# nelaturuharsha/TurboPrune

Measured on NVIDIA H100. Metric: images_per_sec_resnet50_erk80_train_step, higher is better.
Workload: dtype bf16

## Files before the change

turboprune_b200/csrc/tp_igemm.cu:

```cuda
#include "tp_common.cuh"
#include "tp_ptx.cuh"
#include <cuda.h>
#include <mutex>

namespace tp {
using namespace ptx;

constexpr int kBlockM = 128;
constexpr int kBlockK = 64;
constexpr int kConsumers = 256;
constexpr int kThreads = kConsumers + 32;
constexpr int kProducerWarp = kConsumers / 32;
constexpr int kMaxTaps = 64;

__host__ __device__ constexpr int fwd_stages(int block_n) { return block_n == 128 ? 4 : 6; }
__host__ __device__ constexpr int fwd_tail(int block_n) { return kBlockM * block_n * 4 + 8 * 32 * 128 + 1024 + 512; }

struct TapEntry { uint16_t off_w, off_h; int32_t kofs; };

constexpr int kMaxCls = 4;

struct ClsEntry {
  int M;
  int P_it, Q_it;
  int ntaps, tap0;
  int base_w, base_h;
  int oah, oaw;
  int tile0, m_groups;
};

struct FwdParams {
  int M, N;
  int ncls;
  ClsEntry cls[kMaxCls];
  int cchunks;
  int a_mode;
  int step_w, step_h;
  long long out_img_pix;
  int out_row_pix;
// ... 70 lines not shown
  const int ntile = p.m_tiles * p.n_tiles;
  w.split = item / ntile;
  const int tile = item - w.split * ntile, n_t = tile / p.m_tiles;
  w.set_tile(tile - n_t * p.m_tiles, n_t, p.m_tiles, nb, p.chunks);
  w.kb0 = w.split * p.kb_per_split; w.kb1 = min(p.kblocks, w.kb0 + p.kb_per_split);
  return w;
}

__device__ __forceinline__ void decompose_pixel(int m, int P, int Q, int& n, int& p, int& q) {
  q = m % Q; int t = m / Q; p = t % P; n = t / P;
}

struct AMaps { CUtensorMap m[kMaxCls]; };

__device__ __forceinline__ void decode_tile(const FwdParams& p, int tile, int n_tiles, int& c, int& m_g, int& n_t) {
  c = 0;
#pragma unroll
  for (int j = 1; j < kMaxCls; ++j) if (j < p.ncls && tile >= p.cls[j].tile0) c = j;
  const int local = tile - p.cls[c].tile0;
  m_g = local / n_tiles; n_t = local - m_g * n_tiles;
}

template <int BLOCK_N>
__device__ __forceinline__ void fwd_mma_block(float (&acc)[BLOCK_N / 2], uint32_t a_addr, uint32_t b_addr, uint32_t accumulate) {
  const uint64_t adesc = make_smem_desc(a_addr, 16, 1024);
  const uint64_t bdesc = make_smem_desc(b_addr, 16, 1024);
#pragma unroll
  for (int k = 0; k < kBlockK / 16; ++k) {
    if constexpr (BLOCK_N == 128) wgmma_m64n128<0, 0>(acc, adesc + (uint64_t)(2 * k), bdesc + (uint64_t)(2 * k), accumulate | (uint32_t)k);
    else wgmma_m64n64<0, 0>(acc, adesc + (uint64_t)(2 * k), bdesc + (uint64_t)(2 * k), accumulate | (uint32_t)k);
  }
}

template <int BLOCK_N, bool MULTI, bool BNB>
__global__ void __launch_bounds__(kThreads, 1)
k_igemm_fwd(const __grid_constant__ AMaps tmA, const __grid_constant__ CUtensorMap tmB,
            const __grid_constant__ FwdParams p) {
  static_assert(BLOCK_N == 64 || BLOCK_N == 128, "wgmma N of the fwd kernel");
  static_assert(!BNB || !MULTI, "BatchNorm-backward epilogue: single class");
  constexpr int kABytes = kBlockM * kBlockK * 2;
  constexpr int kBBytes = BLOCK_N * kBlockK * 2;
  constexpr int kStageBytes = kABytes + kBBytes;
  constexpr int kStages = fwd_stages(BLOCK_N);
  extern __shared__ __align__(1024) uint8_t smem_raw[];
  uint8_t* smem = (uint8_t*)(((uintptr_t)smem_raw + 1023) & ~(uintptr_t)1023);
  pdl_trigger();
  constexpr int kStgBytes = 32 * 128;
  float* const acc_tile = (float*)(smem + kStages * kStageBytes);
  uint8_t* stg_base = (uint8_t*)(acc_tile + kBlockM * BLOCK_N);
  uint64_t* full_bar = (uint64_t*)(stg_base + 8 * kStgBytes);
  uint64_t* empty_bar = full_bar + kStages;

  const int warp = threadIdx.x >> 5, lane = threadIdx.x & 31;
  const int n_tiles = (p.N + BLOCK_N - 1) / BLOCK_N;
  const int total_tiles = p.cls[p.ncls - 1].tile0 + p.cls[p.ncls - 1].m_groups * n_tiles;
  const int my_items = total_tiles > (int)blockIdx.x ? (total_tiles - (int)blockIdx.x + (int)gridDim.x - 1) / (int)gridDim.x : 0;
  auto get_tile = [&](int w, int& ci, int& m_g, int& n_t) {
    ci = 0;
    const int tile = (int)blockIdx.x + w * (int)gridDim.x;
    if (MULTI) decode_tile(p, tile, n_tiles, ci, m_g, n_t);
    else { m_g = tile / n_tiles; n_t = tile - m_g * n_tiles; }
  };

  if (threadIdx.x == 0) {
    for (int j = 0; j < p.ncls; ++j) prefetch_tmap(&tmA.m[j]);
    prefetch_tmap(&tmB);
    for (int i = 0; i < kStages; ++i) { mbar_init(&full_bar[i], 1); mbar_init(&empty_bar[i], kConsumers / 128); }
    fence_mbar_init();
  }
  __syncthreads();
  pdl_wait();

  if (warp == kProducerWarp) {
    if (lane == 0) {
      int stage = 0; uint32_t phase = 0;
      const uint32_t* const km = live_kmask(p.kmask, p.kmask_words, p.N);
      for (int w = 0; w < my_items; ++w) {
        int ci, m_g, n_t; get_tile(w, ci, m_g, n_t);
        const ClsEntry& ce = p.cls[MULTI ? ci : 0];
        const CUtensorMap* const mapA = &tmA.m[MULTI ? ci : 0];
        const int m0 = m_g * kBlockM;
        int cn = 0, cp = 0, cq = 0;
        if (p.a_mode == 1) decompose_pixel(m0, ce.P_it, ce.Q_it, cn, cp, cq);
        const int cw = ce.base_w + cq * p.step_w, ch = ce.base_h + cp * p.step_h;
        auto load_block = [&](const TapEntry& te, int cc) {
          mbar_wait(&empty_bar[stage], phase ^ 1);
          uint8_t* sA = smem + stage * kStageBytes;
          uint8_t* sB = sA + kABytes;
          mbar_arrive_expect_tx(&full_bar[stage], kStageBytes);
          if (p.a_mode == 1)
            tma_load_im2col_4d(sA, mapA, &full_bar[stage], cc * kBlockK, cw, ch, cn, te.off_w, te.off_h);
          else
            tma_load_2d(sA, mapA, &full_bar[stage], te.kofs + cc * kBlockK, m0);
          tma_load_2d(sB, &tmB, &full_bar[stage], te.kofs + cc * kBlockK, n_t * BLOCK_N);
          if (++stage == kStages) { stage = 0; phase ^= 1; }
        };
        const int tap_base = MULTI ? ce.tap0 : 0;
        if (!km) {
          for (int tap = 0; tap < ce.ntaps; ++tap) {
            const TapEntry te = p.taps[tap_base + tap];
            for (int cc = 0; cc < p.cchunks; ++cc) load_block(te, cc);
          }
        } else {
          KSkip ks; bool any = false;
          ks.begin(km, p.kmask_words, n_t * BLOCK_N, BLOCK_N, p.N);
          for (int tap = 0; tap < ce.ntaps; ++tap) {
            const TapEntry te = p.taps[tap_base + tap];
            for (int cc = 0; cc < p.cchunks; ++cc) {
              const bool last = tap == ce.ntaps - 1 && cc == p.cchunks - 1;
              if (!ks.take((te.kofs >> 6) + cc, last, any)) continue;
              any = true;
              load_block(te, cc);
            }
          }
        }
      }
    }
  } else {
    const int wg = warp >> 2;
    const int quarter = warp & 3;
    const int half = warp >> 2;
    const int erow = quarter * 32 + lane;
    int stage = 0; uint32_t phase = 0;
    const uint32_t* const km = live_kmask(p.kmask, p.kmask_words, p.N);
    auto acc_row_ld = [&](int c, uint32_t* v) {
      const uint32_t rb = smem_u32(acc_tile) + (uint32_t)(erow * BLOCK_N * 4);
#pragma unroll
      for (int i = 0; i < 8; ++i) {
        const uint4 t = lds128(rb + ((uint32_t)(((c >> 2) + i) ^ (erow & 7)) << 4));
        v[4 * i] = t.x; v[4 * i + 1] = t.y; v[4 * i + 2] = t.z; v[4 * i + 3] = t.w;
      }
    };
    for (int w = 0; w < my_items; ++w) {
      int ci, m_g, n_t; get_tile(w, ci, m_g, n_t);
      const ClsEntry& ce = p.cls[MULTI ? ci : 0];
      const bool has_acc = MULTI ? ce.ntaps > 0 : true;
      const int m_t = m_g;
      const int row = m_t * kBlockM + quarter * 32 + lane;
      const bool row_ok = row < ce.M;
      long long opix = 0;
      if (row_ok && !p.staged_store) {
        opix = row;
        if (MULTI || !p.linear) {
          int n, pp, qq; decompose_pixel(row, ce.P_it, ce.Q_it, n, pp, qq);
          opix = (long long)n * p.out_img_pix + (long long)(pp * p.osh + ce.oah) * p.out_row_pix + (qq * p.osw + ce.oaw);
        }
      }
      __nv_bfloat16* orow = p.out + opix * p.ldc;
      const int r_in = lane >> 3, c16 = lane & 7;
      const long long wrow0 = (long long)m_t * kBlockM + quarter * 32;
      const int rows_left = (int)(ce.M - wrow0 < 32 ? (ce.M - wrow0 < 0 ? 0 : ce.M - wrow0) : 32);
      const long long ldc = p.ldc;
      const int N = p.N;
      long long ooff[MULTI ? 8 : 1];
      const long long rbase = (wrow0 + r_in) * ldc + c16 * 8;
      if (MULTI && p.staged_store) {
        int n, pp, qq; decompose_pixel((int)(wrow0 + r_in), ce.P_it, ce.Q_it, n, pp, qq);
#pragma unroll
        for (int i = 0; i < 8; ++i) {
          const long long px = (long long)n * p.out_img_pix + (long long)(pp * p.osh + ce.oah) * p.out_row_pix + (qq * p.osw + ce.oaw);
          ooff[i] = px * ldc + c16 * 8;
          qq += 4;
          while (qq >= ce.Q_it) { qq -= ce.Q_it; if (++pp == ce.P_it) { pp = 0; ++n; } }
        }
      }
      auto row_off = [&](int i) -> long long { return MULTI ? ooff[MULTI ? i : 0] : rbase + (long long)(i * 4) * ldc; };
      if (MULTI && !has_acc) {
        if (p.staged_store) {
#pragma unroll 1
          for (int c = half * 64; c < BLOCK_N; c += 128) {
            const int n0 = n_t * BLOCK_N + c;
            if (n0 >= N) break;
            if (n0 + c16 * 8 + 8 > N) continue;
            uint4 z[8];
#pragma unroll
            for (int i = 0; i < 8; ++i) {
              z[i] = make_uint4(0u, 0u, 0u, 0u);
              if (p.addend && i * 4 + r_in < rows_left) z[i] = *reinterpret_cast<const uint4*>(p.addend + row_off(i) + n0);
            }
#pragma unroll
            for (int i = 0; i < 8; ++i)
              if (i * 4 + r_in < rows_left) *reinterpret_cast<uint4*>(p.out + row_off(i) + n0) = z[i];
          }
        } else if (row_ok && half == 0) {
          for (int j = n_t * BLOCK_N; j < min(p.N, (n_t + 1) * BLOCK_N); ++j)
            orow[j] = p.addend ? p.addend[opix * p.ldc + j] : __float2bfloat16_rn(0.f);
        }
        continue;
      }
      {
        float acc[BLOCK_N / 2];
#pragma unroll
        for (int i = 0; i < BLOCK_N / 2; ++i) acc[i] = 0.f;
        int prev = -1;
        auto mma_block = [&](uint32_t accumulate) {
          mbar_wait(&full_bar[stage], phase);
          const uint32_t s_addr = smem_u32(smem + stage * kStageBytes);
          wgmma_fence();
          fwd_mma_block<BLOCK_N>(acc, s_addr + (uint32_t)(wg * (kABytes / 2)), s_addr + kABytes, accumulate);
          wgmma_commit();
          wgmma_wait<1>();
          if (prev >= 0 && (threadIdx.x & 127) == 0) mbar_arrive(&empty_bar[prev]);
          prev = stage;
          if (++stage == kStages) { stage = 0; phase ^= 1; }
        };
        KSkip ks; uint32_t any = 0;
        if (km) ks.begin(km, p.kmask_words, n_t * BLOCK_N, BLOCK_N, p.N);
        for (int tap = 0; tap < ce.ntaps; ++tap) {
          const int kb0 = p.taps[(MULTI ? ce.tap0 : 0) + tap].kofs >> 6;
          for (int cc = 0; cc < p.cchunks; ++cc) {
            const bool last = tap == ce.ntaps - 1 && cc == p.cchunks - 1;
            if (km && !ks.take(kb0 + cc, last, any)) continue;
            mma_block(any);
            any = 1;
          }
        }
        wgmma_wait<0>();
        acc_fence(acc);
        if (prev >= 0 && (threadIdx.x & 127) == 0) mbar_arrive(&empty_bar[prev]);
        bar_sync(1, kConsumers);
        const int r0 = wg * 64 + (warp & 3) * 16 + (lane >> 2);
#pragma unroll
        for (int j = 0; j < BLOCK_N / 8; ++j)
#pragma unroll
          for (int h = 0; h < 2; ++h) {
            const int r = r0 + 8 * h, col = 8 * j + 2 * (lane & 3);
            *reinterpret_cast<float2*>(acc_tile + r * BLOCK_N + (((col >> 2) ^ (r & 7)) << 2) + (col & 3)) =
                make_float2(acc[4 * j + 2 * h], acc[4 * j + 2 * h + 1]);
          }
        bar_sync(1, kConsumers);
      }
      if (p.staged_store) {
        const uint32_t buf = smem_u32(stg_base + warp * kStgBytes);
        __nv_bfloat16* const gout = p.out;
        const __nv_bfloat16* const gadd = p.addend;
        const float* bias = p.bias;
        float* stats = p.stats ? p.stats + (long long)(m_t * 4 + quarter) * 2 * N + c16 * 8 : nullptr;
        const uint32_t wr_base = buf + lane * 128;
        const uint32_t wr_sw = (uint32_t)(lane & 7);
        const uint32_t rd_even = buf + r_in * 128 + ((uint32_t)(c16 ^ r_in) << 4);
        const uint32_t rd_odd = buf + (r_in + 4) * 128 + ((uint32_t)(c16 ^ (r_in + 4)) << 4);
        uint4 a_pref[8];
#pragma unroll 1
        for (int c = half * 64; c < BLOCK_N; c += 128) {
          const int n0 = n_t * BLOCK_N + c;
          if (n0 >= N) break;
          const bool col_ok = n0 + c16 * 8 + 8 <= N;
          uint32_t v[64];
          acc_row_ld(c, v);
          acc_row_ld(c + 32, v + 32);
          if (gadd) {
            if (c == half * 64) {
#pragma unroll
              for (int i = 0; i < 8; ++i) {
                a_pref[i] = make_uint4(0u, 0u, 0u, 0u);
                if (i * 4 + r_in < rows_left && col_ok) a_pref[i] = *reinterpret_cast<const uint4*>(gadd + row_off(i) + n0);
              }
            }
#pragma unroll
            for (int i = 0; i < 8; ++i) sts128(((i & 1) ? rd_odd : rd_even) + (uint32_t)((i >> 1) * 1024), a_pref[i]);
            if (c + 128 < BLOCK_N && n0 + 128 < N) {
              const bool col_ok2 = n0 + 128 + c16 * 8 + 8 <= N;
#pragma unroll
              for (int i = 0; i < 8; ++i) {
                a_pref[i] = make_uint4(0u, 0u, 0u, 0u);
                if (i * 4 + r_in < rows_left && col_ok2) a_pref[i] = *reinterpret_cast<const uint4*>(gadd + row_off(i) + n0 + 128);
              }
            }
            __syncwarp();
          }
#pragma unroll
          for (int j = 0; j < 64; j += 8) {
            float f[8];
#pragma unroll
            for (int q = 0; q < 8; ++q) f[q] = __uint_as_float(v[j + q]);
            if (bias) {
#pragma unroll
              for (int q = 0; q < 8; ++q) if (n0 + j + q < N) f[q] += bias[n0 + j + q];
            }
            const uint32_t waddr = wr_base + (((uint32_t)(j >> 3) ^ wr_sw) << 4);
            if (gadd) {
              const uint4 a = lds128(waddr);
              const __nv_bfloat162* ah = reinterpret_cast<const __nv_bfloat162*>(&a);
#pragma unroll
              for (int q = 0; q < 4; ++q) { const float2 t2 = __bfloat1622float2(ah[q]); f[2 * q] += t2.x; f[2 * q + 1] += t2.y; }
            }
            __nv_bfloat162 h0 = __floats2bfloat162_rn(f[0], f[1]);
            __nv_bfloat162 h1 = __floats2bfloat162_rn(f[2], f[3]);
            __nv_bfloat162 h2 = __floats2bfloat162_rn(f[4], f[5]);
            __nv_bfloat162 h3 = __floats2bfloat162_rn(f[6], f[7]);
            uint4 pk;
            pk.x = *(uint32_t*)&h0; pk.y = *(uint32_t*)&h1; pk.z = *(uint32_t*)&h2; pk.w = *(uint32_t*)&h3;
            sts128(waddr, pk);
          }
          __syncwarp();
          uint4 o[8];
#pragma unroll
          for (int i = 0; i < 8; ++i) o[i] = lds128(((i & 1) ? rd_odd : rd_even) + (uint32_t)((i >> 1) * 1024));
          float s1[8], s2[8];
#pragma unroll
          for (int q = 0; q < 8; ++q) { s1[q] = 0.f; s2[q] = 0.f; }
          if (BNB) {
            uint4 yv[8];
#pragma unroll
            for (int i = 0; i < 8; ++i) {
              yv[i] = make_uint4(0u, 0u, 0u, 0u);
              if (i * 4 + r_in < rows_left && col_ok) yv[i] = *reinterpret_cast<const uint4*>(p.bn_y + row_off(i) + n0);
            }
            float sc[8], sf[8], is_[8], nm[8];
            if (col_ok) {
              const int cb = n0 + c16 * 8;
#pragma unroll
              for (int q = 0; q < 8; q += 4) {
                const float4 one4 = make_float4(1.f, 1.f, 1.f, 1.f), zero4 = make_float4(0.f, 0.f, 0.f, 0.f);
                const float4 a4 = p.bn_weight ? *reinterpret_cast<const float4*>(p.bn_weight + cb + q) : one4;
                const float4 b4 = p.bn_bias ? *reinterpret_cast<const float4*>(p.bn_bias + cb + q) : zero4;
                const float4 m4 = *reinterpret_cast<const float4*>(p.bn_mean + cb + q), i4 = *reinterpret_cast<const float4*>(p.bn_invstd + cb + q);
                is_[q] = i4.x; is_[q + 1] = i4.y; is_[q + 2] = i4.z; is_[q + 3] = i4.w;
                nm[q] = m4.x; nm[q + 1] = m4.y; nm[q + 2] = m4.z; nm[q + 3] = m4.w;
                sc[q] = a4.x * i4.x; sc[q + 1] = a4.y * i4.y; sc[q + 2] = a4.z * i4.z; sc[q + 3] = a4.w * i4.w;
                sf[q] = fmaf(-m4.x, sc[q], b4.x); sf[q + 1] = fmaf(-m4.y, sc[q + 1], b4.y);
                sf[q + 2] = fmaf(-m4.z, sc[q + 2], b4.z); sf[q + 3] = fmaf(-m4.w, sc[q + 3], b4.w);
              }
            } else {
#pragma unroll
              for (int q = 0; q < 8; ++q) { sc[q] = 0.f; sf[q] = 0.f; is_[q] = 0.f; nm[q] = 0.f; }
            }
#pragma unroll
            for (int i = 0; i < 8; ++i) {
              if (i * 4 + r_in < rows_left) {
                __nv_bfloat162* gh = reinterpret_cast<__nv_bfloat162*>(&o[i]);
                const __nv_bfloat162* yh = reinterpret_cast<const __nv_bfloat162*>(&yv[i]);
#pragma unroll
                for (int q = 0; q < 4; ++q) {
                  float2 d2 = __bfloat1622float2(gh[q]);
                  const float2 y2 = __bfloat1622float2(yh[q]);
                  if (!(fmaf(y2.x, sc[2 * q], sf[2 * q]) > 0.f)) d2.x = 0.f;
                  if (!(fmaf(y2.y, sc[2 * q + 1], sf[2 * q + 1]) > 0.f)) d2.y = 0.f;
                  gh[q] = __floats2bfloat162_rn(d2.x, d2.y);
                  s1[2 * q] += d2.x;     s2[2 * q] = fmaf(d2.x, (y2.x - nm[2 * q]) * is_[2 * q], s2[2 * q]);
                  s1[2 * q + 1] += d2.y; s2[2 * q + 1] = fmaf(d2.y, (y2.y - nm[2 * q + 1]) * is_[2 * q + 1], s2[2 * q + 1]);
                }
              }
            }
          }
#pragma unroll
          for (int i = 0; i < 8; ++i)
            if (i * 4 + r_in < rows_left && col_ok) *reinterpret_cast<uint4*>(gout + row_off(i) + n0) = o[i];
          if (!BNB && stats) {
#pragma unroll
            for (int i = 0; i < 8; ++i) {
              if (i * 4 + r_in < rows_left) {
                const __nv_bfloat162* h2 = reinterpret_cast<const __nv_bfloat162*>(&o[i]);
#pragma unroll
                for (int q = 0; q < 4; ++q) {
                  const float2 t2 = __bfloat1622float2(h2[q]);
                  s1[2 * q] += t2.x; s2[2 * q] = fmaf(t2.x, t2.x, s2[2 * q]);
                  s1[2 * q + 1] += t2.y; s2[2 * q + 1] = fmaf(t2.y, t2.y, s2[2 * q + 1]);
                }
              }
            }
          }
          if (BNB || stats) {
#pragma unroll
            for (int q = 0; q < 8; ++q) {
              s1[q] += __shfl_xor_sync(0xffffffffu, s1[q], 8);  s2[q] += __shfl_xor_sync(0xffffffffu, s2[q], 8);
              s1[q] += __shfl_xor_sync(0xffffffffu, s1[q], 16); s2[q] += __shfl_xor_sync(0xffffffffu, s2[q], 16);
            }
            if (r_in == 0 && col_ok) {
              float4* d1 = reinterpret_cast<float4*>(stats + n0);
              float4* d2 = reinterpret_cast<float4*>(stats + N + n0);
              d1[0] = make_float4(s1[0], s1[1], s1[2], s1[3]); d1[1] = make_float4(s1[4], s1[5], s1[6], s1[7]);
              d2[0] = make_float4(s2[0], s2[1], s2[2], s2[3]); d2[1] = make_float4(s2[4], s2[5], s2[6], s2[7]);
            }
          }
          __syncwarp();
        }
      } else {
#pragma unroll 1
      for (int c = half * 32; c < BLOCK_N; c += 64) {
        uint32_t v[32];
        acc_row_ld(c, v);
        const int n0 = n_t * BLOCK_N + c;
        if (row_ok && n0 < p.N) {
          float f[32];
#pragma unroll
          for (int j = 0; j < 32; ++j) f[j] = __uint_as_float(v[j]);
          if (p.bias) {
#pragma unroll
            for (int j = 0; j < 32; ++j) if (n0 + j < p.N) f[j] += p.bias[n0 + j];
          }
          if (p.addend) {
            const __nv_bfloat16* ar = p.addend + opix * p.ldc + n0;
            for (int j = 0; j < 32; ++j) if (n0 + j < p.N) f[j] += __bfloat162float(ar[j]);
          }
          __nv_bfloat16* dst = orow + n0;
          if (n0 + 32 <= p.N && (((uintptr_t)dst) & 15) == 0) {
#pragma unroll
            for (int j = 0; j < 32; j += 8) {
              __nv_bfloat162 h0 = __floats2bfloat162_rn(f[j], f[j + 1]);
              __nv_bfloat162 h1 = __floats2bfloat162_rn(f[j + 2], f[j + 3]);
              __nv_bfloat162 h2 = __floats2bfloat162_rn(f[j + 4], f[j + 5]);
              __nv_bfloat162 h3 = __floats2bfloat162_rn(f[j + 6], f[j + 7]);
              uint4 pk;
              pk.x = *(uint32_t*)&h0; pk.y = *(uint32_t*)&h1; pk.z = *(uint32_t*)&h2; pk.w = *(uint32_t*)&h3;
              *(uint4*)(dst + j) = pk;
            }
          } else {
            for (int j = 0; j < 32; ++j) if (n0 + j < p.N) dst[j] = __float2bfloat16_rn(f[j]);
          }
        }
      }
      }
    }
  }
}

template <int NB>
__device__ __forceinline__ void wgrad_mma_block(float (&acc)[NB * 32], uint32_t a_addr, uint32_t b_addr, bool first) {
  constexpr uint32_t kChunk = 64 * kBlockK * 2;
#pragma unroll
  for (int k = 0; k < kBlockK / 16; ++k) {
    const uint32_t acc_on = (!first || k > 0) ? 1u : 0u;
    const uint64_t adesc = make_smem_desc(a_addr + (uint32_t)(2048 * k), kChunk, 1024);
    const uint32_t bk = b_addr + (uint32_t)(2048 * k);
    if constexpr (NB >= 2) wgmma_m64n128<1, 1>(acc, adesc, make_smem_desc(bk, kChunk, 1024), acc_on);
    else wgmma_m64n64<1, 1>(acc, adesc, make_smem_desc(bk, kChunk, 1024), acc_on);
    if constexpr (NB == 4) wgmma_m64n128<1, 1>(acc + 64, adesc, make_smem_desc(bk + 2 * kChunk, kChunk, 1024), acc_on);
    if constexpr (NB == 3) wgmma_m64n64<1, 1>(acc + 64, adesc, make_smem_desc(bk + 2 * kChunk, kChunk, 1024), acc_on);
  }
}

template <int NB>
__global__ void __launch_bounds__(kThreads, 1)
k_igemm_wgrad(const __grid_constant__ CUtensorMap tmA ,
// ... 317 lines not shown
  }
}

static int pick_block_n(long long m_tiles, int n) {
  const int sms = sm_count();
  int best = 64; double best_score = -1;
  const int cands[2] = {128, 64};
  const double weight[2] = {1.0, 0.82};
  for (int i = 0; i < 2; ++i) {
    int bn = cands[i];
    if (bn > 64 && n <= bn / 2) continue;
    long long tiles = m_tiles * ((n + bn - 1) / bn);
    long long waves = (tiles + sms - 1) / sms;
    double eff = (double)tiles / (double)(waves * sms) * weight[i];
    if (eff > best_score) { best_score = eff; best = bn; }
  }
  return best;
}

constexpr int kSmemMax = 232448;

template <int BN, bool MULTI, bool BNB = false>
static int launch_fwd(const AMaps& a, const CUtensorMap& b, FwdParams& p, cudaStream_t st) {
  constexpr int smem = fwd_stages(BN) * (kBlockM * kBlockK * 2 + BN * kBlockK * 2) + fwd_tail(BN);
  static_assert(smem <= kSmemMax, "fwd smem budget");
  const int n_tiles = (p.N + BN - 1) / BN;
  static bool attr_set = false;
  if (!attr_set) {
    TP_CUDA_CHECK(cudaFuncSetAttribute(k_igemm_fwd<BN, MULTI, BNB>, cudaFuncAttributeMaxDynamicSharedMemorySize, smem));
    attr_set = true;
  }
  long long ctiles = 0;
  for (int c = 0; c < p.ncls; ++c) {
    p.cls[c].m_groups = (int)((p.cls[c].M + kBlockM - 1) / kBlockM);
    if (ctiles > 0x7fffffffll) return TP_ERR_UNSUPPORTED;
    p.cls[c].tile0 = (int)ctiles;
    ctiles += (long long)p.cls[c].m_groups * n_tiles;
  }
  if (ctiles > 0x7fffffffll || ctiles <= 0) return TP_ERR_UNSUPPORTED;
  const int grid = (int)(ctiles < sm_count() ? ctiles : sm_count());
  TP_CUDA_CHECK(launch(k_igemm_fwd<BN, MULTI, BNB>, dim3(grid), dim3(kThreads), (size_t)smem, st, a, b, p));
  TP_LAUNCH_CHECK();
  return TP_OK;
}

static int run_fwd(const AMaps& a, const CUtensorMap& b, FwdParams& p, int bn, cudaStream_t st) {
  p.linear = p.ncls == 1 && p.osh == 1 && p.osw == 1 && p.cls[0].oah == 0 && p.cls[0].oaw == 0 &&
             p.out_row_pix == p.cls[0].Q_it && p.out_img_pix == (long long)p.cls[0].P_it * p.cls[0].Q_it;
  p.staged_store = (p.ldc % 8 == 0 && p.N % 8 == 0 && (((uintptr_t)p.out) & 15) == 0 &&
                    (!p.addend || (((uintptr_t)p.addend) & 15) == 0)) ? 1 : 0;
  if (p.stats && !(p.staged_store && p.linear)) return TP_ERR_UNSUPPORTED;
  const bool multi = !p.linear;
  if (multi) {
    if (bn == 128) return launch_fwd<128, true>(a, b, p, st);
    return launch_fwd<64, true>(a, b, p, st);
  }
  if (p.bn_y) {
    if (!p.staged_store || !p.stats) return TP_ERR_UNSUPPORTED;
    if (bn == 128) return launch_fwd<128, false, true>(a, b, p, st);
    return launch_fwd<64, false, true>(a, b, p, st);
  }
  if (bn == 128) return launch_fwd<128, false>(a, b, p, st);
  return launch_fwd<64, false>(a, b, p, st);
}
// ... 260 lines not shown
```

turboprune_b200/csrc/tp_ptx.cuh:

```cuda
#pragma once
#include <cuda.h>
#include <cuda_runtime.h>
#include <stdint.h>

namespace tp { namespace ptx {

__device__ __forceinline__ uint32_t smem_u32(const void* p) {
  return (uint32_t)__cvta_generic_to_shared(p);
}

__device__ __forceinline__ void mbar_init(uint64_t* bar, uint32_t count) {
  asm volatile("mbarrier.init.shared::cta.b64 [%0], %1;" :: "r"(smem_u32(bar)), "r"(count) : "memory");
}
__device__ __forceinline__ void fence_mbar_init() {
  asm volatile("fence.mbarrier_init.release.cluster;" ::: "memory");
}
__device__ __forceinline__ void fence_proxy_async() {
  asm volatile("fence.proxy.async.shared::cta;" ::: "memory");
}
__device__ __forceinline__ void mbar_arrive_expect_tx(uint64_t* bar, uint32_t bytes) {
  asm volatile("mbarrier.arrive.expect_tx.shared::cta.b64 _, [%0], %1;" :: "r"(smem_u32(bar)), "r"(bytes) : "memory");
}
__device__ __forceinline__ void mbar_arrive(uint64_t* bar) {
  asm volatile("mbarrier.arrive.shared::cta.b64 _, [%0];" :: "r"(smem_u32(bar)) : "memory");
// ... 3 lines not shown
  asm volatile(
      "{\n\t.reg .pred p;\n\t"
      "mbarrier.try_wait.parity.shared::cta.b64 p, [%1], %2;\n\t"
      "selp.u32 %0, 1, 0, p;\n\t}"
      : "=r"(ok) : "r"(smem_u32(bar)), "r"(parity) : "memory");
  return ok != 0;
}
__device__ __forceinline__ void mbar_wait(uint64_t* bar, uint32_t parity) {
  if (mbar_try_wait(bar, parity)) return;
  long long t0 = clock64();
  while (!mbar_try_wait(bar, parity)) {
    if (clock64() - t0 > 4000000000ll) __trap();
  }
}

__device__ __forceinline__ void sts128(uint32_t addr, const uint4& v) {
  asm volatile("st.shared.v4.b32 [%0], {%1, %2, %3, %4};" :: "r"(addr), "r"(v.x), "r"(v.y), "r"(v.z), "r"(v.w) : "memory");
}
__device__ __forceinline__ uint4 lds128(uint32_t addr) {
  uint4 v;
  asm volatile("ld.shared.v4.b32 {%0, %1, %2, %3}, [%4];" : "=r"(v.x), "=r"(v.y), "=r"(v.z), "=r"(v.w) : "r"(addr) : "memory");
  return v;
}

__device__ __forceinline__ void prefetch_tmap(const CUtensorMap* m) {
  asm volatile("prefetch.tensormap [%0];" :: "l"(m) : "memory");
}
__device__ __forceinline__ void tma_load_2d(void* dst, const CUtensorMap* map, uint64_t* bar, int c0, int c1) {
  asm volatile(
      "cp.async.bulk.tensor.2d.shared::cluster.global.mbarrier::complete_tx::bytes [%0], [%1, {%3, %4}], [%2];"
      :: "r"(smem_u32(dst)), "l"(map), "r"(smem_u32(bar)), "r"(c0), "r"(c1) : "memory");
}
__device__ __forceinline__ void tma_load_im2col_4d(void* dst, const CUtensorMap* map, uint64_t* bar,
                                                   int c, int w, int h, int n, uint16_t off_w, uint16_t off_h) {
  asm volatile(
      "cp.async.bulk.tensor.4d.shared::cluster.global.im2col.mbarrier::complete_tx::bytes"
      " [%0], [%1, {%3, %4, %5, %6}], [%2], {%7, %8};"
      :: "r"(smem_u32(dst)), "l"(map), "r"(smem_u32(bar)), "r"(c), "r"(w), "r"(h), "r"(n), "h"(off_w), "h"(off_h)
      : "memory");
}

__device__ __forceinline__ uint64_t make_smem_desc(uint32_t smem_addr, uint32_t lbo_bytes, uint32_t sbo_bytes) {
  return (uint64_t)((smem_addr & 0x3FFFFu) >> 4) |
         ((uint64_t)((lbo_bytes >> 4) & 0x3FFFu) << 16) |
         ((uint64_t)((sbo_bytes >> 4) & 0x3FFFu) << 32) |
         (1ull << 62);
// ... 66 lines not shown
```

Measured before the change: 6330.

## Ping-pong two consumer warpgroups over full tiles in implicit-GEMM forward

The forward implicit-GEMM kernel now uses a producer warpgroup plus two consumer warpgroups. Each consumer computes a full 128-row tile with two wgmma issues per k-step, and the two alternate tiles via an order barrier that hands over the smem ring position. This lets one warpgroup's epilogue overlap the other's MMA mainloop. Registers are rebalanced with setmaxnreg, stage counts go up, and the fp32 accumulator staging tile is replaced by a per-warpgroup bf16 staging buffer written directly from fragments. The cost is more complex ordering logic and higher register pressure from the doubled accumulator, which risks spills.

Result: faster. 6798 (median of 6 runs) (+7.4%).

```diff
diff --git a/turboprune_b200/csrc/tp_igemm.cu b/turboprune_b200/csrc/tp_igemm.cu
--- a/turboprune_b200/csrc/tp_igemm.cu
+++ b/turboprune_b200/csrc/tp_igemm.cu
@@ -11,10 +11,17 @@
 constexpr int kConsumers = 256;
 constexpr int kThreads = kConsumers + 32;
 constexpr int kProducerWarp = kConsumers / 32;
+constexpr int kFwdThreads = 3 * 128;
 constexpr int kMaxTaps = 64;
 
-__host__ __device__ constexpr int fwd_stages(int block_n) { return block_n == 128 ? 4 : 6; }
-__host__ __device__ constexpr int fwd_tail(int block_n) { return kBlockM * block_n * 4 + 8 * 32 * 128 + 1024 + 512; }
+constexpr int kFwdProducerRegs = 56, kFwdConsumerRegs = 224;
+static_assert(kFwdProducerRegs * 128 + kFwdConsumerRegs * 256 <= 168 * kFwdThreads, "fwd register split");
+
+__host__ __device__ constexpr int fwd_stages(int block_n) { return block_n == 128 ? 5 : 8; }
+__host__ __device__ constexpr int fwd_stg_bytes(int block_n) { return kBlockM * block_n * 2; }
+__host__ __device__ constexpr int fwd_smem(int block_n) {
+  return fwd_stages(block_n) * (kBlockM * kBlockK * 2 + block_n * kBlockK * 2) + 2 * fwd_stg_bytes(block_n) + 1024 + 512;
+}
 
 struct TapEntry { uint16_t off_w, off_h; int32_t kofs; };
 
@@ -131,18 +138,24 @@
 }
 
 template <int BLOCK_N>
-__device__ __forceinline__ void fwd_mma_block(float (&acc)[BLOCK_N / 2], uint32_t a_addr, uint32_t b_addr, uint32_t accumulate) {
+__device__ __forceinline__ void fwd_mma_block(float (&acc)[BLOCK_N], uint32_t a_addr, uint32_t b_addr, uint32_t accumulate) {
   const uint64_t adesc = make_smem_desc(a_addr, 16, 1024);
+  const uint64_t adesc_hi = make_smem_desc(a_addr + 64 * kBlockK * 2, 16, 1024);
   const uint64_t bdesc = make_smem_desc(b_addr, 16, 1024);
 #pragma unroll
   for (int k = 0; k < kBlockK / 16; ++k) {
-    if constexpr (BLOCK_N == 128) wgmma_m64n128<0, 0>(acc, adesc + (uint64_t)(2 * k), bdesc + (uint64_t)(2 * k), accumulate | (uint32_t)k);
-    else wgmma_m64n64<0, 0>(acc, adesc + (uint64_t)(2 * k), bdesc + (uint64_t)(2 * k), accumulate | (uint32_t)k);
+    if constexpr (BLOCK_N == 128) {
+      wgmma_m64n128<0, 0>(acc, adesc + (uint64_t)(2 * k), bdesc + (uint64_t)(2 * k), accumulate | (uint32_t)k);
+      wgmma_m64n128<0, 0>(acc + BLOCK_N / 2, adesc_hi + (uint64_t)(2 * k), bdesc + (uint64_t)(2 * k), accumulate | (uint32_t)k);
+    } else {
+      wgmma_m64n64<0, 0>(acc, adesc + (uint64_t)(2 * k), bdesc + (uint64_t)(2 * k), accumulate | (uint32_t)k);
+      wgmma_m64n64<0, 0>(acc + BLOCK_N / 2, adesc_hi + (uint64_t)(2 * k), bdesc + (uint64_t)(2 * k), accumulate | (uint32_t)k);
+    }
   }
 }
 
 template <int BLOCK_N, bool MULTI, bool BNB>
-__global__ void __launch_bounds__(kThreads, 1)
+__global__ void __launch_bounds__(kFwdThreads, 1)
 k_igemm_fwd(const __grid_constant__ AMaps tmA, const __grid_constant__ CUtensorMap tmB,
             const __grid_constant__ FwdParams p) {
   static_assert(BLOCK_N == 64 || BLOCK_N == 128, "wgmma N of the fwd kernel");
@@ -154,11 +167,13 @@
   extern __shared__ __align__(1024) uint8_t smem_raw[];
   uint8_t* smem = (uint8_t*)(((uintptr_t)smem_raw + 1023) & ~(uintptr_t)1023);
   pdl_trigger();
-  constexpr int kStgBytes = 32 * 128;
-  float* const acc_tile = (float*)(smem + kStages * kStageBytes);
-  uint8_t* stg_base = (uint8_t*)(acc_tile + kBlockM * BLOCK_N);
-  uint64_t* full_bar = (uint64_t*)(stg_base + 8 * kStgBytes);
+  constexpr int kStgBytes = fwd_stg_bytes(BLOCK_N);
+  constexpr int kChunkStg = kBlockM * 64 * 2;
+  uint8_t* const stg_base = smem + kStages * kStageBytes;
+  uint64_t* full_bar = (uint64_t*)(stg_base + 2 * kStgBytes);
   uint64_t* empty_bar = full_bar + kStages;
+  uint64_t* order_bar = empty_bar + kStages;
+  int* ring_pos = (int*)(order_bar + 2);
 
   const int warp = threadIdx.x >> 5, lane = threadIdx.x & 31;
   const int n_tiles = (p.N + BLOCK_N - 1) / BLOCK_N;
@@ -174,14 +189,16 @@
   if (threadIdx.x == 0) {
     for (int j = 0; j < p.ncls; ++j) prefetch_tmap(&tmA.m[j]);
     prefetch_tmap(&tmB);
-    for (int i = 0; i < kStages; ++i) { mbar_init(&full_bar[i], 1); mbar_init(&empty_bar[i], kConsumers / 128); }
+    for (int i = 0; i < kStages; ++i) { mbar_init(&full_bar[i], 1); mbar_init(&empty_bar[i], 1); }
+    mbar_init(&order_bar[0], 1); mbar_init(&order_bar[1], 1);
     fence_mbar_init();
   }
   __syncthreads();
   pdl_wait();
 
-  if (warp == kProducerWarp) {
-    if (lane == 0) {
+  if (warp < 4) {
+    setmaxnreg_dec<kFwdProducerRegs>();
+    if (threadIdx.x == 0) {
       int stage = 0; uint32_t phase = 0;
       const uint32_t* const km = live_kmask(p.kmask, p.kmask_words, p.N);
       for (int w = 0; w < my_items; ++w) {
@@ -226,90 +243,50 @@
       }
     }
   } else {
-    const int wg = warp >> 2;
-    const int quarter = warp & 3;
-    const int half = warp >> 2;
-    const int erow = quarter * 32 + lane;
-    int stage = 0; uint32_t phase = 0;
+    setmaxnreg_inc<kFwdConsumerRegs>();
+    const int cw = (warp >> 2) - 1;
+    const int q = warp & 3;
+    const int wtid = threadIdx.x & 127;
+    const int bar_id = 1 + cw;
     const uint32_t* const km = live_kmask(p.kmask, p.kmask_words, p.N);
-    auto acc_row_ld = [&](int c, uint32_t* v) {
-      const uint32_t rb = smem_u32(acc_tile) + (uint32_t)(erow * BLOCK_N * 4);
-#pragma unroll
-      for (int i = 0; i < 8; ++i) {
-        const uint4 t = lds128(rb + ((uint32_t)(((c >> 2) + i) ^ (erow & 7)) << 4));
-        v[4 * i] = t.x; v[4 * i + 1] = t.y; v[4 * i + 2] = t.z; v[4 * i + 3] = t.w;
-      }
-    };
-    for (int w = 0; w < my_items; ++w) {
+    const uint32_t stg = smem_u32(stg_base + cw * kStgBytes);
+    const int fr0 = q * 16 + (lane >> 2);
+    const uint32_t fsw = (uint32_t)(lane >> 2);
+    const uint32_t frag_base = stg + (uint32_t)(fr0 * 128 + (lane & 3) * 4);
+    const int r_in = lane >> 3, c16 = lane & 7;
+    const uint32_t buf = stg + (uint32_t)(q * 32 * 128);
+    const uint32_t rd_even = buf + r_in * 128 + ((uint32_t)(c16 ^ r_in) << 4);
+    const uint32_t rd_odd = buf + (r_in + 4) * 128 + ((uint32_t)(c16 ^ (r_in + 4)) << 4);
+    for (int it = 0, w = cw; w < my_items; ++it, w += 2) {
       int ci, m_g, n_t; get_tile(w, ci, m_g, n_t);
       const ClsEntry& ce = p.cls[MULTI ? ci : 0];
       const bool has_acc = MULTI ? ce.ntaps > 0 : true;
       const int m_t = m_g;
-      const int row = m_t * kBlockM + quarter * 32 + lane;
-      const bool row_ok = row < ce.M;
-      long long opix = 0;
-      if (row_ok && !p.staged_store) {
-        opix = row;
-        if (MULTI || !p.linear) {
-          int n, pp, qq; decompose_pixel(row, ce.P_it, ce.Q_it, n, pp, qq);
-          opix = (long long)n * p.out_img_pix + (long long)(pp * p.osh + ce.oah) * p.out_row_pix + (qq * p.osw + ce.oaw);
-        }
+
+      int stage = 0; uint32_t phase = 0;
+      const int turn = it + cw;
+      if (turn > 0) {
+        mbar_wait(&order_bar[cw], (uint32_t)((turn - 1) & 1));
+        const int pos = *(volatile int*)ring_pos;
+        stage = pos >> 1; phase = (uint32_t)(pos & 1);
       }
-      __nv_bfloat16* orow = p.out + opix * p.ldc;
-      const int r_in = lane >> 3, c16 = lane & 7;
-      const long long wrow0 = (long long)m_t * kBlockM + quarter * 32;
-      const int rows_left = (int)(ce.M - wrow0 < 32 ? (ce.M - wrow0 < 0 ? 0 : ce.M - wrow0) : 32);
-      const long long ldc = p.ldc;
-      const int N = p.N;
-      long long ooff[MULTI ? 8 : 1];
-      const long long rbase = (wrow0 + r_in) * ldc + c16 * 8;
-      if (MULTI && p.staged_store) {
-        int n, pp, qq; decompose_pixel((int)(wrow0 + r_in), ce.P_it, ce.Q_it, n, pp, qq);
-#pragma unroll
-        for (int i = 0; i < 8; ++i) {
-          const long long px = (long long)n * p.out_img_pix + (long long)(pp * p.osh + ce.oah) * p.out_row_pix + (qq * p.osw + ce.oaw);
-          ooff[i] = px * ldc + c16 * 8;
-          qq += 4;
-          while (qq >= ce.Q_it) { qq -= ce.Q_it; if (++pp == ce.P_it) { pp = 0; ++n; } }
-        }
-      }
-      auto row_off = [&](int i) -> long long { return MULTI ? ooff[MULTI ? i : 0] : rbase + (long long)(i * 4) * ldc; };
-      if (MULTI && !has_acc) {
-        if (p.staged_store) {
-#pragma unroll 1
-          for (int c = half * 64; c < BLOCK_N; c += 128) {
-            const int n0 = n_t * BLOCK_N + c;
-            if (n0 >= N) break;
-            if (n0 + c16 * 8 + 8 > N) continue;
-            uint4 z[8];
-#pragma unroll
-            for (int i = 0; i < 8; ++i) {
-              z[i] = make_uint4(0u, 0u, 0u, 0u);
-              if (p.addend && i * 4 + r_in < rows_left) z[i] = *reinterpret_cast<const uint4*>(p.addend + row_off(i) + n0);
-            }
-#pragma unroll
-            for (int i = 0; i < 8; ++i)
-              if (i * 4 + r_in < rows_left) *reinterpret_cast<uint4*>(p.out + row_off(i) + n0) = z[i];
-          }
-        } else if (row_ok && half == 0) {
-          for (int j = n_t * BLOCK_N; j < min(p.N, (n_t + 1) * BLOCK_N); ++j)
-            orow[j] = p.addend ? p.addend[opix * p.ldc + j] : __float2bfloat16_rn(0.f);
-        }
-        continue;
-      }
-      {
-        float acc[BLOCK_N / 2];
-#pragma unroll
-        for (int i = 0; i < BLOCK_N / 2; ++i) acc[i] = 0.f;
+      bar_sync(bar_id, 128);
+      auto pass_turn = [&]() {
+        if (wtid == 0) { *(volatile int*)ring_pos = stage * 2 + (int)phase; mbar_arrive(&order_bar[cw ^ 1]); }
+      };
+      float acc[BLOCK_N];
+      if (has_acc) {
+#pragma unroll
+        for (int i = 0; i < BLOCK_N; ++i) acc[i] = 0.f;
         int prev = -1;
         auto mma_block = [&](uint32_t accumulate) {
           mbar_wait(&full_bar[stage], phase);
           const uint32_t s_addr = smem_u32(smem + stage * kStageBytes);
           wgmma_fence();
-          fwd_mma_block<BLOCK_N>(acc, s_addr + (uint32_t)(wg * (kABytes / 2)), s_addr + kABytes, accumulate);
+          fwd_mma_block<BLOCK_N>(acc, s_addr, s_addr + kABytes, accumulate);
           wgmma_commit();
           wgmma_wait<1>();
-          if (prev >= 0 && (threadIdx.x & 127) == 0) mbar_arrive(&empty_bar[prev]);
+          if (prev >= 0 && wtid == 0) mbar_arrive(&empty_bar[prev]);
           prev = stage;
           if (++stage == kStages) { stage = 0; phase ^= 1; }
         };
@@ -324,91 +301,121 @@
             any = 1;
           }
         }
+        pass_turn();
         wgmma_wait<0>();
         acc_fence(acc);
-        if (prev >= 0 && (threadIdx.x & 127) == 0) mbar_arrive(&empty_bar[prev]);
-        bar_sync(1, kConsumers);
-        const int r0 = wg * 64 + (warp & 3) * 16 + (lane >> 2);
-#pragma unroll
-        for (int j = 0; j < BLOCK_N / 8; ++j)
-#pragma unroll
-          for (int h = 0; h < 2; ++h) {
-            const int r = r0 + 8 * h, col = 8 * j + 2 * (lane & 3);
-            *reinterpret_cast<float2*>(acc_tile + r * BLOCK_N + (((col >> 2) ^ (r & 7)) << 2) + (col & 3)) =
-                make_float2(acc[4 * j + 2 * h], acc[4 * j + 2 * h + 1]);
+        if (prev >= 0 && wtid == 0) mbar_arrive(&empty_bar[prev]);
+      } else {
+        pass_turn();
+      }
+
+      const long long wrow0 = (long long)m_t * kBlockM + q * 32;
+      const int rows_left = (int)(ce.M - wrow0 < 32 ? (ce.M - wrow0 < 0 ? 0 : ce.M - wrow0) : 32);
+      const long long ldc = p.ldc;
+      const int N = p.N;
+      long long ooff[MULTI ? 8 : 1];
+      const long long rbase = (wrow0 + r_in) * ldc + c16 * 8;
+      if (MULTI && p.staged_store) {
+        int n, pp, qq; decompose_pixel((int)(wrow0 + r_in), ce.P_it, ce.Q_it, n, pp, qq);
+#pragma unroll
+        for (int i = 0; i < 8; ++i) {
+          const long long px = (long long)n * p.out_img_pix + (long long)(pp * p.osh + ce.oah) * p.out_row_pix + (qq * p.osw + ce.oaw);
+          ooff[i] = px * ldc + c16 * 8;
+          qq += 4;
+          while (qq >= ce.Q_it) { qq -= ce.Q_it; if (++pp == ce.P_it) { pp = 0; ++n; } }
+        }
+      }
+      auto row_off = [&](int i) -> long long { return MULTI ? ooff[MULTI ? i : 0] : rbase + (long long)(i * 4) * ldc; };
+      if (MULTI && !has_acc) {
+        if (p.staged_store) {
+#pragma unroll 1
+          for (int c = 0; c < BLOCK_N; c += 64) {
+            const int n0 = n_t * BLOCK_N + c;
+            if (n0 >= N) break;
+            if (n0 + c16 * 8 + 8 > N) continue;
+            uint4 z[8];
+#pragma unroll
+            for (int i = 0; i < 8; ++i) {
+              z[i] = make_uint4(0u, 0u, 0u, 0u);
+              if (p.addend && i * 4 + r_in < rows_left) z[i] = *reinterpret_cast<const uint4*>(p.addend + row_off(i) + n0);
+            }
+#pragma unroll
+            for (int i = 0; i < 8; ++i)
+              if (i * 4 + r_in < rows_left) *reinterpret_cast<uint4*>(p.out + row_off(i) + n0) = z[i];
           }
-        bar_sync(1, kConsumers);
+        } else {
+          const int row = m_t * kBlockM + wtid;
+          if (row < ce.M) {
+            int n, pp, qq; decompose_pixel(row, ce.P_it, ce.Q_it, n, pp, qq);
+            const long long opix = (long long)n * p.out_img_pix + (long long)(pp * p.osh + ce.oah) * p.out_row_pix + (qq * p.osw + ce.oaw);
+            for (int j = n_t * BLOCK_N; j < min(p.N, (n_t + 1) * BLOCK_N); ++j)
+              p.out[opix * p.ldc + j] = p.addend ? p.addend[opix * p.ldc + j] : __float2bfloat16_rn(0.f);
+          }
+        }
+        continue;
       }
       if (p.staged_store) {
-        const uint32_t buf = smem_u32(stg_base + warp * kStgBytes);
         __nv_bfloat16* const gout = p.out;
         const __nv_bfloat16* const gadd = p.addend;
         const float* bias = p.bias;
-        float* stats = p.stats ? p.stats + (long long)(m_t * 4 + quarter) * 2 * N + c16 * 8 : nullptr;
-        const uint32_t wr_base = buf + lane * 128;
-        const uint32_t wr_sw = (uint32_t)(lane & 7);
-        const uint32_t rd_even = buf + r_in * 128 + ((uint32_t)(c16 ^ r_in) << 4);
-        const uint32_t rd_odd = buf + (r_in + 4) * 128 + ((uint32_t)(c16 ^ (r_in + 4)) << 4);
-        uint4 a_pref[8];
+        float* stats = p.stats ? p.stats + (long long)(m_t * 4 + q) * 2 * N + c16 * 8 : nullptr;
+        if (gadd) {
+          __syncwarp();
+#pragma unroll
+          for (int ch = 0; ch < BLOCK_N / 64; ++ch) {
+            const int n0 = n_t * BLOCK_N + ch * 64;
+            if (n0 >= N) break;
+            const bool col_ok = n0 + c16 * 8 + 8 <= N;
+            uint4 a[8];
+#pragma unroll
+            for (int i = 0; i < 8; ++i) {
+              a[i] = make_uint4(0u, 0u, 0u, 0u);
+              if (i * 4 + r_in < rows_left && col_ok) a[i] = *reinterpret_cast<const uint4*>(gadd + row_off(i) + n0);
+            }
+#pragma unroll
+            for (int i = 0; i < 8; ++i) sts128(((i & 1) ? rd_odd : rd_even) + (uint32_t)(ch * kChunkStg + (i >> 1) * 1024), a[i]);
+          }
+        }
+        bar_sync(bar_id, 128);
+#pragma unroll
+        for (int ch = 0; ch < BLOCK_N / 64; ++ch) {
+          const int n0 = n_t * BLOCK_N + ch * 64;
+          if (n0 >= N) break;
+#pragma unroll
+          for (int mh = 0; mh < 2; ++mh)
+#pragma unroll
+            for (int h = 0; h < 2; ++h)
+#pragma unroll
+              for (int j = 0; j < 8; ++j) {
+                const int i = mh * (BLOCK_N / 2) + 4 * (ch * 8 + j) + 2 * h;
+                float f0 = acc[i], f1 = acc[i + 1];
+                const int n = n0 + 8 * j + 2 * (lane & 3);
+                if (bias) {
+                  if (n < N) f0 += bias[n];
+                  if (n + 1 < N) f1 += bias[n + 1];
+                }
+                const uint32_t addr = frag_base + (uint32_t)(ch * kChunkStg + (64 * mh + 8 * h) * 128) + (((uint32_t)j ^ fsw) << 4);
+                if (gadd) {
+                  const uint32_t a = lds32(addr);
+                  const float2 t2 = __bfloat1622float2(*reinterpret_cast<const __nv_bfloat162*>(&a));
+                  f0 += t2.x; f1 += t2.y;
+                }
+                const __nv_bfloat162 hv = __floats2bfloat162_rn(f0, f1);
+                sts32(addr, *reinterpret_cast<const uint32_t*>(&hv));
+              }
+        }
+        bar_sync(bar_id, 128);
 #pragma unroll 1
-        for (int c = half * 64; c < BLOCK_N; c += 128) {
-          const int n0 = n_t * BLOCK_N + c;
+        for (int ch = 0; ch < BLOCK_N / 64; ++ch) {
+          const int n0 = n_t * BLOCK_N + ch * 64;
           if (n0 >= N) break;
           const bool col_ok = n0 + c16 * 8 + 8 <= N;
-          uint32_t v[64];
-          acc_row_ld(c, v);
-          acc_row_ld(c + 32, v + 32);
-          if (gadd) {
-            if (c == half * 64) {
-#pragma unroll
-              for (int i = 0; i < 8; ++i) {
-                a_pref[i] = make_uint4(0u, 0u, 0u, 0u);
-                if (i * 4 + r_in < rows_left && col_ok) a_pref[i] = *reinterpret_cast<const uint4*>(gadd + row_off(i) + n0);
-              }
-            }
-#pragma unroll
-            for (int i = 0; i < 8; ++i) sts128(((i & 1) ? rd_odd : rd_even) + (uint32_t)((i >> 1) * 1024), a_pref[i]);
-            if (c + 128 < BLOCK_N && n0 + 128 < N) {
-              const bool col_ok2 = n0 + 128 + c16 * 8 + 8 <= N;
-#pragma unroll
-              for (int i = 0; i < 8; ++i) {
-                a_pref[i] = make_uint4(0u, 0u, 0u, 0u);
-                if (i * 4 + r_in < rows_left && col_ok2) a_pref[i] = *reinterpret_cast<const uint4*>(gadd + row_off(i) + n0 + 128);
-              }
-            }
-            __syncwarp();
-          }
-#pragma unroll
-          for (int j = 0; j < 64; j += 8) {
-            float f[8];
-#pragma unroll
-            for (int q = 0; q < 8; ++q) f[q] = __uint_as_float(v[j + q]);
-            if (bias) {
-#pragma unroll
-              for (int q = 0; q < 8; ++q) if (n0 + j + q < N) f[q] += bias[n0 + j + q];
-            }
-            const uint32_t waddr = wr_base + (((uint32_t)(j >> 3) ^ wr_sw) << 4);
-            if (gadd) {
-              const uint4 a = lds128(waddr);
-              const __nv_bfloat162* ah = reinterpret_cast<const __nv_bfloat162*>(&a);
-#pragma unroll
-              for (int q = 0; q < 4; ++q) { const float2 t2 = __bfloat1622float2(ah[q]); f[2 * q] += t2.x; f[2 * q + 1] += t2.y; }
-            }
-            __nv_bfloat162 h0 = __floats2bfloat162_rn(f[0], f[1]);
-            __nv_bfloat162 h1 = __floats2bfloat162_rn(f[2], f[3]);
-            __nv_bfloat162 h2 = __floats2bfloat162_rn(f[4], f[5]);
-            __nv_bfloat162 h3 = __floats2bfloat162_rn(f[6], f[7]);
-            uint4 pk;
-            pk.x = *(uint32_t*)&h0; pk.y = *(uint32_t*)&h1; pk.z = *(uint32_t*)&h2; pk.w = *(uint32_t*)&h3;
-            sts128(waddr, pk);
-          }
-          __syncwarp();
           uint4 o[8];
 #pragma unroll
-          for (int i = 0; i < 8; ++i) o[i] = lds128(((i & 1) ? rd_odd : rd_even) + (uint32_t)((i >> 1) * 1024));
+          for (int i = 0; i < 8; ++i) o[i] = lds128(((i & 1) ? rd_odd : rd_even) + (uint32_t)(ch * kChunkStg + (i >> 1) * 1024));
           float s1[8], s2[8];
 #pragma unroll
-          for (int q = 0; q < 8; ++q) { s1[q] = 0.f; s2[q] = 0.f; }
+          for (int qq = 0; qq < 8; ++qq) { s1[qq] = 0.f; s2[qq] = 0.f; }
           if (BNB) {
             uint4 yv[8];
 #pragma unroll
@@ -420,20 +427,20 @@
             if (col_ok) {
               const int cb = n0 + c16 * 8;
 #pragma unroll
-              for (int q = 0; q < 8; q += 4) {
+              for (int qq = 0; qq < 8; qq += 4) {
                 const float4 one4 = make_float4(1.f, 1.f, 1.f, 1.f), zero4 = make_float4(0.f, 0.f, 0.f, 0.f);
-                const float4 a4 = p.bn_weight ? *reinterpret_cast<const float4*>(p.bn_weight + cb + q) : one4;
-                const float4 b4 = p.bn_bias ? *reinterpret_cast<const float4*>(p.bn_bias + cb + q) : zero4;
-                const float4 m4 = *reinterpret_cast<const float4*>(p.bn_mean + cb + q), i4 = *reinterpret_cast<const float4*>(p.bn_invstd + cb + q);
-                is_[q] = i4.x; is_[q + 1] = i4.y; is_[q + 2] = i4.z; is_[q + 3] = i4.w;
-                nm[q] = m4.x; nm[q + 1] = m4.y; nm[q + 2] = m4.z; nm[q + 3] = m4.w;
-                sc[q] = a4.x * i4.x; sc[q + 1] = a4.y * i4.y; sc[q + 2] = a4.z * i4.z; sc[q + 3] = a4.w * i4.w;
-                sf[q] = fmaf(-m4.x, sc[q], b4.x); sf[q + 1] = fmaf(-m4.y, sc[q + 1], b4.y);
-                sf[q + 2] = fmaf(-m4.z, sc[q + 2], b4.z); sf[q + 3] = fmaf(-m4.w, sc[q + 3], b4.w);
+                const float4 a4 = p.bn_weight ? *reinterpret_cast<const float4*>(p.bn_weight + cb + qq) : one4;
+                const float4 b4 = p.bn_bias ? *reinterpret_cast<const float4*>(p.bn_bias + cb + qq) : zero4;
+                const float4 m4 = *reinterpret_cast<const float4*>(p.bn_mean + cb + qq), i4 = *reinterpret_cast<const float4*>(p.bn_invstd + cb + qq);
+                is_[qq] = i4.x; is_[qq + 1] = i4.y; is_[qq + 2] = i4.z; is_[qq + 3] = i4.w;
+                nm[qq] = m4.x; nm[qq + 1] = m4.y; nm[qq + 2] = m4.z; nm[qq + 3] = m4.w;
+                sc[qq] = a4.x * i4.x; sc[qq + 1] = a4.y * i4.y; sc[qq + 2] = a4.z * i4.z; sc[qq + 3] = a4.w * i4.w;
+                sf[qq] = fmaf(-m4.x, sc[qq], b4.x); sf[qq + 1] = fmaf(-m4.y, sc[qq + 1], b4.y);
+                sf[qq + 2] = fmaf(-m4.z, sc[qq + 2], b4.z); sf[qq + 3] = fmaf(-m4.w, sc[qq + 3], b4.w);
               }
             } else {
 #pragma unroll
-              for (int q = 0; q < 8; ++q) { sc[q] = 0.f; sf[q] = 0.f; is_[q] = 0.f; nm[q] = 0.f; }
+              for (int qq = 0; qq < 8; ++qq) { sc[qq] = 0.f; sf[qq] = 0.f; is_[qq] = 0.f; nm[qq] = 0.f; }
             }
 #pragma unroll
             for (int i = 0; i < 8; ++i) {
@@ -441,14 +448,14 @@
                 __nv_bfloat162* gh = reinterpret_cast<__nv_bfloat162*>(&o[i]);
                 const __nv_bfloat162* yh = reinterpret_cast<const __nv_bfloat162*>(&yv[i]);
 #pragma unroll
-                for (int q = 0; q < 4; ++q) {
-                  float2 d2 = __bfloat1622float2(gh[q]);
-                  const float2 y2 = __bfloat1622float2(yh[q]);
-                  if (!(fmaf(y2.x, sc[2 * q], sf[2 * q]) > 0.f)) d2.x = 0.f;
-                  if (!(fmaf(y2.y, sc[2 * q + 1], sf[2 * q + 1]) > 0.f)) d2.y = 0.f;
-                  gh[q] = __floats2bfloat162_rn(d2.x, d2.y);
-                  s1[2 * q] += d2.x;     s2[2 * q] = fmaf(d2.x, (y2.x - nm[2 * q]) * is_[2 * q], s2[2 * q]);
-                  s1[2 * q + 1] += d2.y; s2[2 * q + 1] = fmaf(d2.y, (y2.y - nm[2 * q + 1]) * is_[2 * q + 1], s2[2 * q + 1]);
+                for (int qq = 0; qq < 4; ++qq) {
+                  float2 d2 = __bfloat1622float2(gh[qq]);
+                  const float2 y2 = __bfloat1622float2(yh[qq]);
+                  if (!(fmaf(y2.x, sc[2 * qq], sf[2 * qq]) > 0.f)) d2.x = 0.f;
+                  if (!(fmaf(y2.y, sc[2 * qq + 1], sf[2 * qq + 1]) > 0.f)) d2.y = 0.f;
+                  gh[qq] = __floats2bfloat162_rn(d2.x, d2.y);
+                  s1[2 * qq] += d2.x;     s2[2 * qq] = fmaf(d2.x, (y2.x - nm[2 * qq]) * is_[2 * qq], s2[2 * qq]);
+                  s1[2 * qq + 1] += d2.y; s2[2 * qq + 1] = fmaf(d2.y, (y2.y - nm[2 * qq + 1]) * is_[2 * qq + 1], s2[2 * qq + 1]);
                 }
               }
             }
@@ -462,19 +469,19 @@
               if (i * 4 + r_in < rows_left) {
                 const __nv_bfloat162* h2 = reinterpret_cast<const __nv_bfloat162*>(&o[i]);
 #pragma unroll
-                for (int q = 0; q < 4; ++q) {
-                  const float2 t2 = __bfloat1622float2(h2[q]);
-                  s1[2 * q] += t2.x; s2[2 * q] = fmaf(t2.x, t2.x, s2[2 * q]);
-                  s1[2 * q + 1] += t2.y; s2[2 * q + 1] = fmaf(t2.y, t2.y, s2[2 * q + 1]);
+                for (int qq = 0; qq < 4; ++qq) {
+                  const float2 t2 = __bfloat1622float2(h2[qq]);
+                  s1[2 * qq] += t2.x; s2[2 * qq] = fmaf(t2.x, t2.x, s2[2 * qq]);
+                  s1[2 * qq + 1] += t2.y; s2[2 * qq + 1] = fmaf(t2.y, t2.y, s2[2 * qq + 1]);
                 }
               }
             }
           }
           if (BNB || stats) {
 #pragma unroll
-            for (int q = 0; q < 8; ++q) {
-              s1[q] += __shfl_xor_sync(0xffffffffu, s1[q], 8);  s2[q] += __shfl_xor_sync(0xffffffffu, s2[q], 8);
-              s1[q] += __shfl_xor_sync(0xffffffffu, s1[q], 16); s2[q] += __shfl_xor_sync(0xffffffffu, s2[q], 16);
+            for (int qq = 0; qq < 8; ++qq) {
+              s1[qq] += __shfl_xor_sync(0xffffffffu, s1[qq], 8);  s2[qq] += __shfl_xor_sync(0xffffffffu, s2[qq], 8);
+              s1[qq] += __shfl_xor_sync(0xffffffffu, s1[qq], 16); s2[qq] += __shfl_xor_sync(0xffffffffu, s2[qq], 16);
             }
             if (r_in == 0 && col_ok) {
               float4* d1 = reinterpret_cast<float4*>(stats + n0);
@@ -483,43 +490,32 @@
               d2[0] = make_float4(s2[0], s2[1], s2[2], s2[3]); d2[1] = make_float4(s2[4], s2[5], s2[6], s2[7]);
             }
           }
-          __syncwarp();
         }
       } else {
-#pragma unroll 1
-      for (int c = half * 32; c < BLOCK_N; c += 64) {
-        uint32_t v[32];
-        acc_row_ld(c, v);
-        const int n0 = n_t * BLOCK_N + c;
-        if (row_ok && n0 < p.N) {
-          float f[32];
-#pragma unroll
-          for (int j = 0; j < 32; ++j) f[j] = __uint_as_float(v[j]);
-          if (p.bias) {
-#pragma unroll
-            for (int j = 0; j < 32; ++j) if (n0 + j < p.N) f[j] += p.bias[n0 + j];
+#pragma unroll
+        for (int mh = 0; mh < 2; ++mh)
+#pragma unroll
+          for (int h = 0; h < 2; ++h) {
+            const int row = m_t * kBlockM + fr0 + 8 * h + 64 * mh;
+            if (row >= ce.M) continue;
+            long long opix = row;
+            if (MULTI || !p.linear) {
+              int n, pp, qq; decompose_pixel(row, ce.P_it, ce.Q_it, n, pp, qq);
+              opix = (long long)n * p.out_img_pix + (long long)(pp * p.osh + ce.oah) * p.out_row_pix + (qq * p.osw + ce.oaw);
+            }
+            __nv_bfloat16* const orow = p.out + opix * p.ldc;
+#pragma unroll
+            for (int j = 0; j < BLOCK_N / 8; ++j)
+#pragma unroll
+              for (int e = 0; e < 2; ++e) {
+                const int n = n_t * BLOCK_N + 8 * j + 2 * (lane & 3) + e;
+                if (n >= N) continue;
+                float f = acc[mh * (BLOCK_N / 2) + 4 * j + 2 * h + e];
+                if (p.bias) f += p.bias[n];
+                if (p.addend) f += __bfloat162float(p.addend[opix * p.ldc + n]);
+                orow[n] = __float2bfloat16_rn(f);
+              }
           }
-          if (p.addend) {
-            const __nv_bfloat16* ar = p.addend + opix * p.ldc + n0;
-            for (int j = 0; j < 32; ++j) if (n0 + j < p.N) f[j] += __bfloat162float(ar[j]);
-          }
-          __nv_bfloat16* dst = orow + n0;
-          if (n0 + 32 <= p.N && (((uintptr_t)dst) & 15) == 0) {
-#pragma unroll
-            for (int j = 0; j < 32; j += 8) {
-              __nv_bfloat162 h0 = __floats2bfloat162_rn(f[j], f[j + 1]);
-              __nv_bfloat162 h1 = __floats2bfloat162_rn(f[j + 2], f[j + 3]);
-              __nv_bfloat162 h2 = __floats2bfloat162_rn(f[j + 4], f[j + 5]);
-              __nv_bfloat162 h3 = __floats2bfloat162_rn(f[j + 6], f[j + 7]);
-              uint4 pk;
-              pk.x = *(uint32_t*)&h0; pk.y = *(uint32_t*)&h1; pk.z = *(uint32_t*)&h2; pk.w = *(uint32_t*)&h3;
-              *(uint4*)(dst + j) = pk;
-            }
-          } else {
-            for (int j = 0; j < 32; ++j) if (n0 + j < p.N) dst[j] = __float2bfloat16_rn(f[j]);
-          }
-        }
-      }
       }
     }
   }
@@ -883,7 +879,7 @@
 
 template <int BN, bool MULTI, bool BNB = false>
 static int launch_fwd(const AMaps& a, const CUtensorMap& b, FwdParams& p, cudaStream_t st) {
-  constexpr int smem = fwd_stages(BN) * (kBlockM * kBlockK * 2 + BN * kBlockK * 2) + fwd_tail(BN);
+  constexpr int smem = fwd_smem(BN);
   static_assert(smem <= kSmemMax, "fwd smem budget");
   const int n_tiles = (p.N + BN - 1) / BN;
   static bool attr_set = false;
@@ -900,7 +896,7 @@
   }
   if (ctiles > 0x7fffffffll || ctiles <= 0) return TP_ERR_UNSUPPORTED;
   const int grid = (int)(ctiles < sm_count() ? ctiles : sm_count());
-  TP_CUDA_CHECK(launch(k_igemm_fwd<BN, MULTI, BNB>, dim3(grid), dim3(kThreads), (size_t)smem, st, a, b, p));
+  TP_CUDA_CHECK(launch(k_igemm_fwd<BN, MULTI, BNB>, dim3(grid), dim3(kFwdThreads), (size_t)smem, st, a, b, p));
   TP_LAUNCH_CHECK();
   return TP_OK;
 }
diff --git a/turboprune_b200/csrc/tp_ptx.cuh b/turboprune_b200/csrc/tp_ptx.cuh
--- a/turboprune_b200/csrc/tp_ptx.cuh
+++ b/turboprune_b200/csrc/tp_ptx.cuh
@@ -49,6 +49,19 @@
   asm volatile("ld.shared.v4.b32 {%0, %1, %2, %3}, [%4];" : "=r"(v.x), "=r"(v.y), "=r"(v.z), "=r"(v.w) : "r"(addr) : "memory");
   return v;
 }
+__device__ __forceinline__ void sts32(uint32_t addr, uint32_t v) {
+  asm volatile("st.shared.b32 [%0], %1;" :: "r"(addr), "r"(v) : "memory");
+}
+__device__ __forceinline__ uint32_t lds32(uint32_t addr) {
+  uint32_t v;
+  asm volatile("ld.shared.b32 %0, [%1];" : "=r"(v) : "r"(addr) : "memory");
+  return v;
+}
+
+template <int N>
+__device__ __forceinline__ void setmaxnreg_inc() { asm volatile("setmaxnreg.inc.sync.aligned.u32 %0;" :: "n"(N)); }
+template <int N>
+__device__ __forceinline__ void setmaxnreg_dec() { asm volatile("setmaxnreg.dec.sync.aligned.u32 %0;" :: "n"(N)); }
 
 __device__ __forceinline__ void prefetch_tmap(const CUtensorMap* m) {
   asm volatile("prefetch.tensormap [%0];" :: "l"(m) : "memory");
```
